# tqch/ddpm-torch

Hardware: AMD Instinct MI355X
Metric: training imgs/s/GPU + 1000-step DDPM samples/s, CIFAR-10 UNet @1/2/4/8 MI355X (higher is better)
Workload: dtype bf16; 1 GPU; configs/cifar10.json UNet (35.7M params), full Trainer.step, B=128 per GPU, 32x32, T=1000, dropout 0.1, Adam+clip+EMA; global_batch=128, rccl_ranks=1, parallelism=dp1

## Files before the change

### ddpm-torch_amd/csrc/optim.hip

```cpp
#include "common.h"

__global__ void sumsq_kernel(const float* __restrict__ g, long long n, float* __restrict__ partial) {
    __shared__ float sh[4];
    float acc = 0.f;
    for (long long i = (long long)blockIdx.x * blockDim.x + threadIdx.x; i < n; i += (long long)gridDim.x * blockDim.x) acc += g[i] * g[i];
    acc = wave_sum(acc);
    if ((threadIdx.x & 63) == 0) sh[threadIdx.x >> 6] = acc;
    __syncthreads();
    if (threadIdx.x == 0) partial[blockIdx.x] = sh[0] + sh[1] + sh[2] + sh[3];
}
__global__ void sum_partials_kernel(const float* __restrict__ partial, int nblk, float* __restrict__ out) {
    __shared__ float sh[4];
    float acc = 0.f;
    for (int i = threadIdx.x; i < nblk; i += blockDim.x) acc += partial[i];
    acc = wave_sum(acc);
    if ((threadIdx.x & 63) == 0) sh[threadIdx.x >> 6] = acc;
    __syncthreads();
    if (threadIdx.x == 0) out[0] += sh[0] + sh[1] + sh[2] + sh[3];
}
extern "C" int ddpm_sumsq_accumulate(const float* g, long long n, float* total_sq, float* workspace, void* stream) {
    if (!g || !total_sq || !workspace) return DDPM_ERR_NULL;
    if (n <= 0) return DDPM_OK;
    long long want = (n + 255) / 256;
    const int nblk = (int)(want > 1024 ? 1024 : want);
    hipLaunchKernelGGL(sumsq_kernel, dim3(nblk), dim3(256), 0, (hipStream_t)stream, g, n, workspace);
    hipLaunchKernelGGL(sum_partials_kernel, dim3(1), dim3(256), 0, (hipStream_t)stream, workspace, nblk, total_sq);
    return check_launch();
}

__global__ void adam_ema_kernel(float* __restrict__ p, const float* __restrict__ g, float* __restrict__ m, float* __restrict__ v,
                                float* __restrict__ shadow, long long n, const float* __restrict__ total_sq, float max_norm,
                                float lr, float beta1, float beta2, float eps, float bc1, float bc2, float ema_w) {
    float clip = 1.f;
    if (total_sq && max_norm > 0.f) {
        const float c = max_norm / (sqrtf(total_sq[0]) + 1e-6f);
        clip = c < 1.f ? c : 1.f;
    }
    const float step = lr / bc1;
    const float sqrt_bc2 = sqrtf(bc2);
    for (long long i = (long long)blockIdx.x * blockDim.x + threadIdx.x; i < n; i += (long long)gridDim.x * blockDim.x) {
        const float gi = g[i] * clip;
        const float mi = beta1 * m[i] + (1.f - beta1) * gi;
        const float vi = beta2 * v[i] + (1.f - beta2) * gi * gi;
        m[i] = mi; v[i] = vi;
        const float denom = sqrtf(vi) / sqrt_bc2 + eps;
        const float pi = p[i] - step * (mi / denom);
        p[i] = pi;
        if (shadow) shadow[i] += ema_w * (pi - shadow[i]);
    }
}
extern "C" int ddpm_adam_ema_step(float* p, const float* g, float* m, float* v, float* shadow, long long n, const float* total_sq,
                                  float max_norm, float lr, float beta1, float beta2, float eps, float bias_corr1, float bias_corr2,
                                  float ema_w, void* stream) {
    if (!p || !g || !m || !v) return DDPM_ERR_NULL;
    if (n <= 0) return DDPM_OK;
    long long want = (n + 255) / 256;
    const int nblk = (int)(want > 4096 ? 4096 : want);
    hipLaunchKernelGGL(adam_ema_kernel, dim3(nblk), dim3(256), 0, (hipStream_t)stream, p, g, m, v, shadow, n, total_sq, max_norm, lr, beta1, beta2,
                       eps, bias_corr1, bias_corr2, ema_w);
    return check_launch();
}

constexpr int MT_SUMSQ_LANES = 64;
__global__ __launch_bounds__(1024) void sumsq_finish_kernel(const float* __restrict__ partial, int n, float* __restrict__ total_sq) {
    __shared__ float sh[1024];
    float acc = 0.f;
    for (int i = threadIdx.x; i < n; i += 1024) acc += partial[i];
    sh[threadIdx.x] = acc;
    __syncthreads();
    for (int w = 512; w > 0; w >>= 1) {
        if ((int)threadIdx.x < w) sh[threadIdx.x] += sh[threadIdx.x + w];
        __syncthreads();
    }
    if (threadIdx.x < MT_SUMSQ_LANES) total_sq[threadIdx.x] = threadIdx.x == 0 ? sh[0] : 0.f;
}
int ddpm_sumsq_finish_launch(const float* partial, int n, float* total_sq, void* stream) {
    hipLaunchKernelGGL(sumsq_finish_kernel, dim3(1), dim3(1024), 0, (hipStream_t)stream, partial, n, total_sq);
    return check_launch();
}
constexpr int MT_SUMSQ_BLOCKS = 16;
__global__ void mt_sumsq_kernel(const long long* __restrict__ table, float* __restrict__ partial) {
    __shared__ float sh[4];
    const long long* row = table + 6 * (long long)blockIdx.y;
    const float* g = reinterpret_cast<const float*>(row[1]);
    const long long n = row[5];
    float acc = 0.f;
    const long long nv = (reinterpret_cast<unsigned long long>(g) & 15) == 0 ? n >> 2 : 0;
    for (long long i = (long long)blockIdx.x * blockDim.x + threadIdx.x; i < nv; i += (long long)gridDim.x * blockDim.x) {
        const float4 v = reinterpret_cast<const float4*>(g)[i];
        acc += (v.x * v.x + v.y * v.y) + (v.z * v.z + v.w * v.w);
    }
    for (long long i = (nv << 2) + (long long)blockIdx.x * blockDim.x + threadIdx.x; i < n; i += (long long)gridDim.x * blockDim.x) acc += g[i] * g[i];
    acc = wave_sum(acc);
    if ((threadIdx.x & 63) == 0) sh[threadIdx.x >> 6] = acc;
    __syncthreads();
    if (threadIdx.x == 0) partial[blockIdx.y * gridDim.x + blockIdx.x] = (sh[0] + sh[1]) + (sh[2] + sh[3]);
}
__global__ void mt_adam_ema_kernel(const long long* __restrict__ table, const float* __restrict__ total_sq, float max_norm, float lr,
                                   float beta1, float beta2, float eps, float bc1, float bc2, float ema_w, const float* __restrict__ hyper) {
    if (hyper) { lr = hyper[0]; bc1 = hyper[1]; bc2 = hyper[2]; ema_w = hyper[3]; }
    const long long* row = table + 6 * (long long)blockIdx.y;
    float* p = reinterpret_cast<float*>(row[0]);
    const float* g = reinterpret_cast<const float*>(row[1]);
    float* m = reinterpret_cast<float*>(row[2]);
    float* v = reinterpret_cast<float*>(row[3]);
    float* shadow = reinterpret_cast<float*>(row[4]);
    const long long n = row[5];
    float clip = 1.f;
    if (total_sq && max_norm > 0.f) {
        float tot = 0.f;
        for (int i = 0; i < MT_SUMSQ_LANES; ++i) tot += total_sq[i];
        const float c = max_norm / (sqrtf(tot) + 1e-6f);
        clip = c < 1.f ? c : 1.f;
    }
    const float step = lr / bc1;
    const float sqrt_bc2 = sqrtf(bc2);
    auto upd = [&](float& pi, float gi, float& mi, float& vi, float& si) {
        gi *= clip;
        mi = beta1 * mi + (1.f - beta1) * gi;
        vi = beta2 * vi + (1.f - beta2) * gi * gi;
        const float denom = sqrtf(vi) / sqrt_bc2 + eps;
        pi = pi - step * (mi / denom);
        si += ema_w * (pi - si);
    };
    const unsigned long long al = reinterpret_cast<unsigned long long>(p) | reinterpret_cast<unsigned long long>(g) | reinterpret_cast<unsigned long long>(m) |
                                  reinterpret_cast<unsigned long long>(v) | reinterpret_cast<unsigned long long>(shadow);
    const long long nv = (al & 15) == 0 ? n >> 2 : 0;
    for (long long i = (long long)blockIdx.x * blockDim.x + threadIdx.x; i < nv; i += (long long)gridDim.x * blockDim.x) {
        float4 p4 = reinterpret_cast<float4*>(p)[i], m4 = reinterpret_cast<float4*>(m)[i], v4 = reinterpret_cast<float4*>(v)[i];
        const float4 g4 = reinterpret_cast<const float4*>(g)[i];
        float4 s4 = shadow ? reinterpret_cast<float4*>(shadow)[i] : make_float4(0.f, 0.f, 0.f, 0.f);
        upd(p4.x, g4.x, m4.x, v4.x, s4.x); upd(p4.y, g4.y, m4.y, v4.y, s4.y);
        upd(p4.z, g4.z, m4.z, v4.z, s4.z); upd(p4.w, g4.w, m4.w, v4.w, s4.w);
        reinterpret_cast<float4*>(p)[i] = p4; reinterpret_cast<float4*>(m)[i] = m4; reinterpret_cast<float4*>(v)[i] = v4;
        if (shadow) reinterpret_cast<float4*>(shadow)[i] = s4;
    }
    for (long long i = (nv << 2) + (long long)blockIdx.x * blockDim.x + threadIdx.x; i < n; i += (long long)gridDim.x * blockDim.x) {
        float pi = p[i], mi = m[i], vi = v[i], si = shadow ? shadow[i] : 0.f;
        upd(pi, g[i], mi, vi, si);
        p[i] = pi; m[i] = mi; v[i] = vi;
        if (shadow) shadow[i] = si;
    }
}
extern "C" int ddpm_mt_sumsq_slots(int n_tensors) { return MT_SUMSQ_LANES + 64 * (n_tensors > 0 ? n_tensors : 0); }
extern "C" int ddpm_mt_grad_sumsq(const long long* table, int n_tensors, float* total_sq, long long total_sq_floats, void* stream) {
    if (!table || !total_sq) return DDPM_ERR_NULL;
    if (n_tensors <= 0) return DDPM_OK;
    if (total_sq_floats < ddpm_mt_sumsq_slots(n_tensors)) return DDPM_ERR_SHAPE;
    hipLaunchKernelGGL(mt_sumsq_kernel, dim3(MT_SUMSQ_BLOCKS, n_tensors), dim3(256), 0, (hipStream_t)stream, table, total_sq + MT_SUMSQ_LANES);
    const int rc = check_launch();
    return rc ? rc : ddpm_sumsq_finish_launch(total_sq + MT_SUMSQ_LANES, MT_SUMSQ_BLOCKS * n_tensors, total_sq, stream);
}
extern "C" int ddpm_mt_adam_ema(const long long* table, int n_tensors, const float* total_sq, float max_norm, float lr, float beta1,
                                float beta2, float eps, float bias_corr1, float bias_corr2, float ema_w, const float* hyper_dev, void* stream) {
    if (!table) return DDPM_ERR_NULL;
    if (n_tensors <= 0) return DDPM_OK;
    hipLaunchKernelGGL(mt_adam_ema_kernel, dim3(32, n_tensors), dim3(256), 0, (hipStream_t)stream, table, total_sq, max_norm, lr, beta1, beta2, eps,
                       bias_corr1, bias_corr2, ema_w, hyper_dev);
    return check_launch();
}
```

### ddpm-torch_amd/csrc/wgrad1x1.hip

```cpp
#include "common.h"
#include <string.h>
#include <stdlib.h>

namespace {

typedef __bf16 bf16x8 __attribute__((ext_vector_type(8)));
typedef float f32x4v __attribute__((ext_vector_type(4)));

struct Wg1Args {
    const bf16_t* dy; long long dy_ld; unsigned dy_extent;
    const bf16_t* x; long long x_ld; unsigned x_extent;
    float* dw; long long slab_stride;
    float* dbias; long long bias_stride;
    int P, C, N, tiles_c, tiles_n, ksteps, ksteps_per_split;
};

constexpr int RING = 4, OP_BYTES = 64 * 256, STAGE = 2 * OP_BYTES;
constexpr int PER = 4;

template <int N> __device__ __forceinline__ void wait_vm() {
    static_assert(N >= 0 && N < 64, "vmcnt immediate");
    asm volatile("s_waitcnt vmcnt(%0)" :: "n"(N) : "memory");
}

__global__ __launch_bounds__(512, 2)
void wgrad1x1_kernel(Wg1Args a) {
    extern __shared__ __attribute__((aligned(16))) char smem[];
    const int tid = threadIdx.x, lane = tid & 63;
    const int wave = __builtin_amdgcn_readfirstlane(tid >> 6);
    const int wc = wave & 1, wn = wave >> 1;
    const int ntiles = a.tiles_c * a.tiles_n;
    const int split = blockIdx.x / ntiles, tile = blockIdx.x - split * ntiles;
    const int tn = tile / a.tiles_c, tc = tile - tn * a.tiles_c;
    const int ks0 = split * a.ksteps_per_split, nst = max(min(a.ksteps, ks0 + a.ksteps_per_split) - ks0, 0);

    auto rsrc_of = [&](const void* p, unsigned extent) {
        const unsigned long long ad = (unsigned long long)p;
        const unsigned lo = __builtin_amdgcn_readfirstlane((unsigned)ad), hi = __builtin_amdgcn_readfirstlane((unsigned)(ad >> 32));
        return __builtin_amdgcn_make_buffer_rsrc(reinterpret_cast<void*>(((unsigned long long)hi << 32) | lo), 0,
                                                 __builtin_amdgcn_readfirstlane((int)extent), 0x00020000);
    };
    const __amdgpu_buffer_rsrc_t rdy = rsrc_of(a.dy, a.dy_extent), rx = rsrc_of(a.x, a.x_extent);

    unsigned xoff[2], yoff[2];
#pragma unroll
    for (int i = 0; i < 2; ++i) {
        const int v = tid + 512 * i, row = v >> 4, lc = (v & 15) ^ ((row & 3) << 2);
        const int c = tc * 128 + lc * 8, n = tn * 128 + lc * 8;
        xoff[i] = c < a.C ? (unsigned)(((long long)row * a.x_ld + c) * 2) : 0x7ffffff0u;
        yoff[i] = n < a.N ? (unsigned)(((long long)row * a.dy_ld + n) * 2) : 0x7ffffff0u;
    }
    const unsigned x_step = (unsigned)(64 * a.x_ld * 2), y_step = (unsigned)(64 * a.dy_ld * 2);
    auto issue = [&](int st) {
        char* dst = smem + (st & (RING - 1)) * STAGE;
        const unsigned kx = (unsigned)(ks0 + st) * x_step, ky = (unsigned)(ks0 + st) * y_step;
#pragma unroll
        for (int i = 0; i < 2; ++i)
            __builtin_amdgcn_raw_ptr_buffer_load_lds(rx, (__attribute__((address_space(3))) void*)(dst + (wave * 64 + 512 * i) * 16), 16,
                                                     xoff[i] == 0x7ffffff0u ? xoff[i] : xoff[i] + kx, 0, 0, 0);
#pragma unroll
        for (int i = 0; i < 2; ++i)
            __builtin_amdgcn_raw_ptr_buffer_load_lds(rdy, (__attribute__((address_space(3))) void*)(dst + OP_BYTES + (wave * 64 + 512 * i) * 16), 16,
                                                     yoff[i] == 0x7ffffff0u ? yoff[i] : yoff[i] + ky, 0, 0, 0);
    };

    const int i16 = lane & 15;
    auto frag_off = [&](int rb, int kc) {
        const int mcol = rb + ((lane >> 4) & 1) * 16 + (i16 & 3) * 4;
        const int krow = kc * 16 + (lane >> 5) * 8 + (i16 >> 2);
        const int pch = (mcol >> 3) ^ ((krow & 3) << 2);
        return (unsigned)(krow * 256 + pch * 16 + (mcol & 7) * 2);
    };
    unsigned offA[2], offB;
    offA[0] = frag_off(wc * 64, 0); offA[1] = frag_off(wc * 64 + 32, 0);
    offB = frag_off(wn * 32, 0) + OP_BYTES;
    const unsigned lds0 = (unsigned)(size_t)smem;

    f32x16 acc[2] = {(f32x16)(0.f), (f32x16)(0.f)};
    float bsum = 0.f;
    const bool want_bias = a.dbias != nullptr && tc == 0 && wc == 0;

#pragma unroll
    for (int t = 0; t < RING - 1; ++t)
        if (t < nst) issue(t);

    for (int st = 0; st < nst; ++st) {
        const int newer = min(RING - 2, nst - 1 - st);
        if (newer >= 2) wait_vm<2 * PER>(); else if (newer == 1) wait_vm<PER>(); else wait_vm<0>();
        __builtin_amdgcn_s_barrier();
        if (st + RING - 1 < nst) issue(st + RING - 1);
        const unsigned base = lds0 + (st & (RING - 1)) * STAGE;
        uint2 fa[4][2][2], fb[4][2];
#pragma unroll
        for (int kc = 0; kc < 4; ++kc) {
#pragma unroll
            for (int i = 0; i < 2; ++i) {
                asm volatile("ds_read_b64_tr_b16 %0, %1 offset:%2" : "=v"(fa[kc][i][0]) : "v"(base + offA[i]), "n"(kc * 4096) : "memory");
                asm volatile("ds_read_b64_tr_b16 %0, %1 offset:%2" : "=v"(fa[kc][i][1]) : "v"(base + offA[i]), "n"(kc * 4096 + 1024) : "memory");
            }
            asm volatile("ds_read_b64_tr_b16 %0, %1 offset:%2" : "=v"(fb[kc][0]) : "v"(base + offB), "n"(kc * 4096) : "memory");
            asm volatile("ds_read_b64_tr_b16 %0, %1 offset:%2" : "=v"(fb[kc][1]) : "v"(base + offB), "n"(kc * 4096 + 1024) : "memory");
        }
        asm volatile("s_waitcnt lgkmcnt(0)" ::: "memory");
        __builtin_amdgcn_sched_barrier(0);
#pragma unroll
        for (int kc = 0; kc < 4; ++kc) {
            const u32x4 vb = {fb[kc][0].x, fb[kc][0].y, fb[kc][1].x, fb[kc][1].y};
#pragma unroll
            for (int i = 0; i < 2; ++i) {
                const u32x4 va = {fa[kc][i][0].x, fa[kc][i][0].y, fa[kc][i][1].x, fa[kc][i][1].y};
                acc[i] = __builtin_amdgcn_mfma_f32_32x32x16_bf16(__builtin_bit_cast(bf16x8, va), __builtin_bit_cast(bf16x8, vb), acc[i], 0, 0, 0);
            }
            if (want_bias)
                bsum += __uint_as_float(vb.x << 16) + __uint_as_float(vb.x & 0xffff0000u) + __uint_as_float(vb.y << 16) + __uint_as_float(vb.y & 0xffff0000u)
                      + __uint_as_float(vb.z << 16) + __uint_as_float(vb.z & 0xffff0000u) + __uint_as_float(vb.w << 16) + __uint_as_float(vb.w & 0xffff0000u);
        }
    }

    const int n = tn * 128 + wn * 32 + (lane & 31);
    float* slab = a.dw + (long long)split * a.slab_stride;
    if (n < a.N) {
#pragma unroll
        for (int i = 0; i < 2; ++i)
#pragma unroll
            for (int g = 0; g < 4; ++g) {
                const int c = tc * 128 + wc * 64 + i * 32 + 8 * g + 4 * (lane >> 5);
                if (c < a.C) {
                    f32x4v o = {acc[i][4 * g], acc[i][4 * g + 1], acc[i][4 * g + 2], acc[i][4 * g + 3]};
                    *reinterpret_cast<f32x4v*>(slab + (long long)n * a.C + c) = o;
                }
            }
    }
    if (want_bias) {
        bsum += __shfl_xor(bsum, 32, 64);
        if (lane < 32 && n < a.N) a.dbias[(long long)split * a.bias_stride + n] = bsum;
    }
}

struct Plan { int tiles_c, tiles_n, ksteps, splits, ksteps_per_split; };
static bool make_plan(int P, int C, int N, Plan& p) {
    if (P <= 0 || C <= 0 || N <= 0 || C % 8 || N % 8) return false;
    p.tiles_c = (C + 127) / 128; p.tiles_n = (N + 127) / 128;
    p.ksteps = (P + 63) / 64;
    const int tiles = p.tiles_c * p.tiles_n;
    constexpr int cu_budget = 128;
    int splits = ddpm_cu_budget(cu_budget) / tiles;
    if (splits < 1) splits = 1;
    const int max_splits = p.ksteps / 4 > 0 ? p.ksteps / 4 : 1;
    if (splits > max_splits) splits = max_splits;
    p.ksteps_per_split = (p.ksteps + splits - 1) / splits;
    p.splits = (p.ksteps + p.ksteps_per_split - 1) / p.ksteps_per_split;
    return true;
}

}

extern "C" int ddpm_conv1x1_wgrad_splits(int P, int C, int N) {
    constexpr int min_p = 2048;
    Plan p;
    if (P < min_p || !make_plan(P, C, N, p)) return 0;
    return p.splits;
}

extern "C" int ddpm_conv1x1_wgrad_nhwc(const void* dy, long long dy_ld, const void* x, long long x_ld, float* dw, long long slab_stride,
                                       float* dbias, long long bias_stride, int P, int C, int N, int splits, int dtype, void* stream) {
    if (!dy || !x || !dw) return DDPM_ERR_NULL;
    if (dtype != DDPM_BF16) return DDPM_ERR_DTYPE;
    Plan p;
    if (!make_plan(P, C, N, p) || splits != p.splits || slab_stride < (long long)N * C || (dbias && bias_stride < N) || dy_ld < N || x_ld < C) return DDPM_ERR_SHAPE;
    if (!aligned16(dy) || !aligned16(x) || !aligned16(dw) || dy_ld % 8 || x_ld % 8 || slab_stride % 4 || C % 4) return DDPM_ERR_ALIGN;
    const long long dyb = ((long long)(P - 1) * dy_ld + N) * 2, xb = ((long long)(P - 1) * x_ld + C) * 2;
    if (dyb > 0x7ffffff0ll || xb > 0x7ffffff0ll) return DDPM_ERR_SHAPE;
    Wg1Args a; memset(&a, 0, sizeof(a));
    a.dy = (const bf16_t*)dy; a.dy_ld = dy_ld; a.dy_extent = (unsigned)dyb;
    a.x = (const bf16_t*)x; a.x_ld = x_ld; a.x_extent = (unsigned)xb;
    a.dw = dw; a.slab_stride = slab_stride; a.dbias = dbias; a.bias_stride = bias_stride;
    a.P = P; a.C = C; a.N = N; a.tiles_c = p.tiles_c; a.tiles_n = p.tiles_n; a.ksteps = p.ksteps; a.ksteps_per_split = p.ksteps_per_split;
    constexpr int LDS = RING * STAGE;
    static DevOnce attr_set;
    if (!attr_set) {
        if (hipFuncSetAttribute(reinterpret_cast<const void*>(&wgrad1x1_kernel), hipFuncAttributeMaxDynamicSharedMemorySize, LDS) != hipSuccess) return DDPM_ERR_LAUNCH;
        attr_set = true;
    }
    hipLaunchKernelGGL(wgrad1x1_kernel, dim3(p.tiles_c * p.tiles_n * p.splits), dim3(512), LDS, (hipStream_t)stream, a);
    return check_launch();
}
```

Measured before the change: 14610 imgs/s.

## Balance multi-tensor Adam over chunks and remap wgrad1x1 blocks per XCD

The fused Adam+EMA kernel no longer launches a fixed 32 blocks per tensor. It builds a per-block prefix sum of 1024-element chunks across all tensors and hands chunks out grid-stride to a persistent grid sized from the CU count, so small and large tensors are spread evenly and idle blocks are avoided. Separately, the 1x1 weight-gradient kernel remaps block indices so consecutive work tiles land on the same XCD, aiming for better L2 reuse. The Adam change adds a redundant per-block scan of the tensor table, which is extra work and shared-memory use in exchange for load balance.

```diff
diff --git a/ddpm-torch_amd/csrc/optim.hip b/ddpm-torch_amd/csrc/optim.hip
--- a/ddpm-torch_amd/csrc/optim.hip
+++ b/ddpm-torch_amd/csrc/optim.hip
@@ -96,16 +96,15 @@
     __syncthreads();
     if (threadIdx.x == 0) partial[blockIdx.y * gridDim.x + blockIdx.x] = (sh[0] + sh[1]) + (sh[2] + sh[3]);
 }
-__global__ void mt_adam_ema_kernel(const long long* __restrict__ table, const float* __restrict__ total_sq, float max_norm, float lr,
-                                   float beta1, float beta2, float eps, float bc1, float bc2, float ema_w, const float* __restrict__ hyper) {
+constexpr int MT_CHUNK = 1024;
+constexpr int MT_SEG = 1024;
+constexpr int MT_ADAM_BLOCKS_PER_CU = 8;
+__global__ __launch_bounds__(256) void mt_adam_ema_kernel(const long long* __restrict__ table, int n_tensors, const float* __restrict__ total_sq,
+                                                          float max_norm, float lr, float beta1, float beta2, float eps, float bc1, float bc2,
+                                                          float ema_w, const float* __restrict__ hyper) {
+    __shared__ long long cstart[MT_SEG + 1];
+    __shared__ long long wtot[4];
     if (hyper) { lr = hyper[0]; bc1 = hyper[1]; bc2 = hyper[2]; ema_w = hyper[3]; }
-    const long long* row = table + 6 * (long long)blockIdx.y;
-    float* p = reinterpret_cast<float*>(row[0]);
-    const float* g = reinterpret_cast<const float*>(row[1]);
-    float* m = reinterpret_cast<float*>(row[2]);
-    float* v = reinterpret_cast<float*>(row[3]);
-    float* shadow = reinterpret_cast<float*>(row[4]);
-    const long long n = row[5];
     float clip = 1.f;
     if (total_sq && max_norm > 0.f) {
         float tot = 0.f;
@@ -123,23 +122,74 @@
         pi = pi - step * (mi / denom);
         si += ema_w * (pi - si);
     };
-    const unsigned long long al = reinterpret_cast<unsigned long long>(p) | reinterpret_cast<unsigned long long>(g) | reinterpret_cast<unsigned long long>(m) |
-                                  reinterpret_cast<unsigned long long>(v) | reinterpret_cast<unsigned long long>(shadow);
-    const long long nv = (al & 15) == 0 ? n >> 2 : 0;
-    for (long long i = (long long)blockIdx.x * blockDim.x + threadIdx.x; i < nv; i += (long long)gridDim.x * blockDim.x) {
-        float4 p4 = reinterpret_cast<float4*>(p)[i], m4 = reinterpret_cast<float4*>(m)[i], v4 = reinterpret_cast<float4*>(v)[i];
-        const float4 g4 = reinterpret_cast<const float4*>(g)[i];
-        float4 s4 = shadow ? reinterpret_cast<float4*>(shadow)[i] : make_float4(0.f, 0.f, 0.f, 0.f);
-        upd(p4.x, g4.x, m4.x, v4.x, s4.x); upd(p4.y, g4.y, m4.y, v4.y, s4.y);
-        upd(p4.z, g4.z, m4.z, v4.z, s4.z); upd(p4.w, g4.w, m4.w, v4.w, s4.w);
-        reinterpret_cast<float4*>(p)[i] = p4; reinterpret_cast<float4*>(m)[i] = m4; reinterpret_cast<float4*>(v)[i] = v4;
-        if (shadow) reinterpret_cast<float4*>(shadow)[i] = s4;
-    }
-    for (long long i = (nv << 2) + (long long)blockIdx.x * blockDim.x + threadIdx.x; i < n; i += (long long)gridDim.x * blockDim.x) {
-        float pi = p[i], mi = m[i], vi = v[i], si = shadow ? shadow[i] : 0.f;
-        upd(pi, g[i], mi, vi, si);
-        p[i] = pi; m[i] = mi; v[i] = vi;
-        if (shadow) shadow[i] = si;
+    const int tid = threadIdx.x, lane = tid & 63, wave = tid >> 6;
+    long long seg_base = 0;
+    long long c = blockIdx.x;
+    for (int r0 = 0; r0 < n_tensors; r0 += MT_SEG) {
+        const int rows = min(MT_SEG, n_tensors - r0);
+        long long cnt[4], mine = 0;
+#pragma unroll
+        for (int j = 0; j < 4; ++j) {
+            const int r = 4 * tid + j;
+            const long long n = r < rows ? table[6 * (long long)(r0 + r) + 5] : 0;
+            cnt[j] = n > 0 ? (n + MT_CHUNK - 1) / MT_CHUNK : 0;
+            mine += cnt[j];
+        }
+        long long inc = mine;
+#pragma unroll
+        for (int d = 1; d < 64; d <<= 1) {
+            const long long o = __shfl_up(inc, d, 64);
+            if (lane >= d) inc += o;
+        }
+        __syncthreads();
+        if (lane == 63) wtot[wave] = inc;
+        __syncthreads();
+        long long before = seg_base + inc - mine;
+        for (int w = 0; w < wave; ++w) before += wtot[w];
+#pragma unroll
+        for (int j = 0; j < 4; ++j) {
+            cstart[4 * tid + j] = before;
+            before += cnt[j];
+        }
+        if (tid == 255) cstart[MT_SEG] = before;
+        __syncthreads();
+        const long long seg_end = cstart[MT_SEG];
+        int r = 0, held = -1;
+        float* p = nullptr; const float* g = nullptr; float* m = nullptr; float* v = nullptr; float* shadow = nullptr;
+        long long n = 0, nv = 0;
+        for (; c < seg_end; c += gridDim.x) {
+            while (cstart[r + 1] <= c) ++r;
+            if (r != held) {
+                const long long* row = table + 6 * (long long)(r0 + r);
+                p = reinterpret_cast<float*>(row[0]); g = reinterpret_cast<const float*>(row[1]);
+                m = reinterpret_cast<float*>(row[2]); v = reinterpret_cast<float*>(row[3]);
+                shadow = reinterpret_cast<float*>(row[4]); n = row[5];
+                const unsigned long long al = reinterpret_cast<unsigned long long>(p) | reinterpret_cast<unsigned long long>(g) |
+                                              reinterpret_cast<unsigned long long>(m) | reinterpret_cast<unsigned long long>(v) |
+                                              reinterpret_cast<unsigned long long>(shadow);
+                nv = (al & 15) == 0 ? n >> 2 : 0;
+                held = r;
+            }
+            const long long e0 = (c - cstart[r]) * MT_CHUNK;
+            const long long i4 = (e0 >> 2) + tid;
+            if (i4 < nv) {
+                float4 p4 = reinterpret_cast<float4*>(p)[i4], m4 = reinterpret_cast<float4*>(m)[i4], v4 = reinterpret_cast<float4*>(v)[i4];
+                const float4 g4 = reinterpret_cast<const float4*>(g)[i4];
+                float4 s4 = shadow ? reinterpret_cast<float4*>(shadow)[i4] : make_float4(0.f, 0.f, 0.f, 0.f);
+                upd(p4.x, g4.x, m4.x, v4.x, s4.x); upd(p4.y, g4.y, m4.y, v4.y, s4.y);
+                upd(p4.z, g4.z, m4.z, v4.z, s4.z); upd(p4.w, g4.w, m4.w, v4.w, s4.w);
+                reinterpret_cast<float4*>(p)[i4] = p4; reinterpret_cast<float4*>(m)[i4] = m4; reinterpret_cast<float4*>(v)[i4] = v4;
+                if (shadow) reinterpret_cast<float4*>(shadow)[i4] = s4;
+            }
+            const long long e1 = min(e0 + MT_CHUNK, n);
+            for (long long i = max(e0, nv << 2) + tid; i < e1; i += 256) {
+                float pi = p[i], mi = m[i], vi = v[i], si = shadow ? shadow[i] : 0.f;
+                upd(pi, g[i], mi, vi, si);
+                p[i] = pi; m[i] = mi; v[i] = vi;
+                if (shadow) shadow[i] = si;
+            }
+        }
+        seg_base = seg_end;
     }
 }
 extern "C" int ddpm_mt_sumsq_slots(int n_tensors) { return MT_SUMSQ_LANES + 64 * (n_tensors > 0 ? n_tensors : 0); }
@@ -155,7 +205,7 @@
                                 float beta2, float eps, float bias_corr1, float bias_corr2, float ema_w, const float* hyper_dev, void* stream) {
     if (!table) return DDPM_ERR_NULL;
     if (n_tensors <= 0) return DDPM_OK;
-    hipLaunchKernelGGL(mt_adam_ema_kernel, dim3(32, n_tensors), dim3(256), 0, (hipStream_t)stream, table, total_sq, max_norm, lr, beta1, beta2, eps,
-                       bias_corr1, bias_corr2, ema_w, hyper_dev);
-    return check_launch();
-}
+    hipLaunchKernelGGL(mt_adam_ema_kernel, dim3(MT_ADAM_BLOCKS_PER_CU * ddpm_cu_budget(256)), dim3(256), 0, (hipStream_t)stream, table, n_tensors, total_sq,
+                       max_norm, lr, beta1, beta2, eps, bias_corr1, bias_corr2, ema_w, hyper_dev);
+    return check_launch();
+}
diff --git a/ddpm-torch_amd/csrc/wgrad1x1.hip b/ddpm-torch_amd/csrc/wgrad1x1.hip
--- a/ddpm-torch_amd/csrc/wgrad1x1.hip
+++ b/ddpm-torch_amd/csrc/wgrad1x1.hip
@@ -30,7 +30,9 @@
     const int wave = __builtin_amdgcn_readfirstlane(tid >> 6);
     const int wc = wave & 1, wn = wave >> 1;
     const int ntiles = a.tiles_c * a.tiles_n;
-    const int split = blockIdx.x / ntiles, tile = blockIdx.x - split * ntiles;
+    const int nblk = gridDim.x, xcd = blockIdx.x & 7;
+    const int w = xcd * (nblk >> 3) + min(xcd, nblk & 7) + (blockIdx.x >> 3);
+    const int split = w / ntiles, tile = w - split * ntiles;
     const int tn = tile / a.tiles_c, tc = tile - tn * a.tiles_c;
     const int ks0 = split * a.ksteps_per_split, nst = max(min(a.ksteps, ks0 + a.ksteps_per_split) - ks0, 0);
 
```

New measurement: 14680 imgs/s, median of 6. About the same (+0.5%).
